# isabella232/kyverno

Hardware: AMD Instinct MI355X
Metric: resource×rule validate evals/sec (node) (higher is better)
Workload: dtype u8; 1 GPU; C2: synthetic Pods x 100 validate.pattern rules (image globs, ?*, quantities, |-lists); rules=100, pairs_per_gpu=100000000, output=full, parallelism=resource-shard x1, engine=specialized

## Files before the change

### kyverno_amd/csrc/kvdevfn.h

```cpp
#pragma once

#define KV_SENT 0xFFFFFFFFu


#ifdef KV_JIT_PRELUDE
#define KV_FN __device__ __forceinline__
#define KV_GLOB_FN __device__ __forceinline__
#else
#define KV_FN __device__
#define KV_GLOB_FN __device__ __noinline__
#endif

__device__ __forceinline__ uint32_t uni(uint32_t v) { return __builtin_amdgcn_readfirstlane(v); }

#ifndef KV_SCONST
#define KV_SCONST __attribute__((address_space(4)))
#endif
template <class T>
__device__ __forceinline__ T sld(const T* p) {
  static_assert(sizeof(T) % 4 == 0, "sld: whole words");
  const KV_SCONST uint32_t* q = (const KV_SCONST uint32_t*)p;
  uint32_t w[sizeof(T) / 4];
#pragma unroll
  for (uint32_t i = 0; i < sizeof(T) / 4; i++) w[i] = q[i];
// ... 576 lines not shown
  if (xm == 1) {
    for (uint32_t f = xf; f < xf + xc; f++)
      if (!(sld(P.fflags + f) & MF_EMPTY) && block_errs(P, B, R, rkind, rflags, f) == 0) return false;
    return true;
  }
  if (xm == 2) {
    for (uint32_t f = xf; f < xf + xc; f++)
      if ((sld(P.fflags + f) & MF_EMPTY) || block_errs(P, B, R, rkind, rflags, f) != 0) return true;
    return false;
  }
  if (!(sld(P.fflags + xf) & MF_EMPTY) && block_errs(P, B, R, rkind, rflags, xf) == 0) return false;
  return true;
}

__device__ __forceinline__ uint32_t wave_min(uint32_t v) {
#pragma unroll
  for (int o = 32; o >= 1; o >>= 1) {
    uint32_t x = __shfl_xor(v, o, 64);
    v = x < v ? x : v;
  }
  return v;
}


struct EState {
  uint32_t kind, flags, pn, key, res, i0, i1, i2, i3;
};

__device__ __forceinline__ uint2 err8_pack(uint32_t kind, uint32_t flags, uint32_t pn, uint32_t key, uint32_t i0,
                                           uint32_t i1, uint32_t i2, uint32_t i3, uint32_t r) {
  const uint32_t fits = (i0 < 1024u) & (i1 < 256u) & (i2 < 256u) & (i3 == 0u) & (key == ABSENT) & (pn < (1u << 25));
  uint2 w;
  w.x = kind | (flags << 4) | ((fits ^ 1u) << 6) | (pn << 7);
  w.y = (i0 & 1023u) | ((i1 & 255u) << 10) | ((i2 & 255u) << 18) | ((r & 63u) << 26);
  return w;
}

__device__ __forceinline__ void store_err(const DevOut& O, uint32_t ri, uint32_t n_res, uint32_t r, uint32_t kind,
                                          uint32_t flags, uint32_t pn, uint32_t key, uint32_t res, uint32_t i0,
                                          uint32_t i1, uint32_t i2, uint32_t i3) {
#if defined(KV_JIT_PRELUDE) && !defined(KVEMU)
  if (KV_OFULL(O) & 4) return;
#else
  if (KV_OFULL(O) & 4) {
    uint4* x = (uint4*)(O.err + (size_t)ri * n_res) + 2u * r;
    x[0] = make_uint4(kind | (flags << 16), pn, key, res);
    x[1] = make_uint4(i0, i1, i2, i3);
    return;
  }
#endif
  ((uint2*)(O.err8 + (size_t)ri * n_res))[r] = err8_pack(kind, flags, pn, key, i0, i1, i2, i3, r);
}

__device__ __forceinline__ uint32_t kv_count_bytes(uint32_t w, uint32_t b4) {
  const uint32_t t = w ^ b4;
  return (uint32_t)__popc(~(((t & 0x7F7F7F7Fu) + 0x7F7F7F7Fu) | t | 0x7F7F7F7Fu));
}

__device__ __forceinline__ uint32_t kv_ptab_col(uint32_t n_vals, uint32_t type, uint32_t a) {
  if (type - 1u < 4u) return a;
  return n_vals - KV_PTAB_PSEUDO + (type == NT_NULL ? 0u : type == NT_MAP ? 1u : 2u);
}
__device__ __forceinline__ uint32_t kv_ptab_col(const DevPS& P, uint32_t type, uint32_t a) {
  return kv_ptab_col(P.n_vals, type, a);
}

__device__ __forceinline__ uint32_t kv_arr_word(const uint32_t* __restrict__ ptab, uint32_t n_vals,
                                                const Node* __restrict__ N, uint32_t first, uint32_t count, uint32_t w) {
  uint32_t x = 0xFFFFFFFFu;
  for (uint32_t k = 0; k < count; k++) {
    const Node e = N[ni(first + k)];
    x &= kv_gld(ptab, (size_t)w * n_vals + kv_ptab_col(n_vals, node_type(e.kt), e.a));
  }
  return x;
}

__device__ __forceinline__ uint32_t kv_leaf_word(const DevPS& P, const Node* __restrict__ N, const Node& n, uint32_t w) {
  const uint32_t t = node_type(n.kt);
#ifdef KV_DIAG_XPTAB
  if (t != NT_ARR) return (n.a * 0x9E3779B9u) ^ (w * 0x85EBCA6Bu);
#endif
  if (t != NT_ARR) return kv_gld(P.ptab, (size_t)w * P.n_vals + kv_ptab_col(P, t, n.a));
  return kv_arr_word(P.ptab, P.n_vals, N, n.a, n.b, w);
}

__device__ __forceinline__ uint32_t kv_leaf_gather(const DevPS& P, const Node& n, uint32_t w) {
#ifdef KV_DIAG_XPTAB
  if (node_type(n.kt) != NT_ARR) return (n.a * 0x9E3779B9u) ^ (w * 0x85EBCA6Bu);
#endif
  return kv_gld(P.ptab, (size_t)w * P.n_vals + kv_ptab_col(P, node_type(n.kt), n.a));
}
__device__ __forceinline__ uint32_t kv_leaf_fix(const uint32_t* __restrict__ ptab, uint32_t n_vals, const Node* __restrict__ N,
                                             uint32_t a, uint32_t b, bool narrow, uint32_t w) {
  if (narrow) {
    const uint32_t ai = ni(a);
    a = kv_gld(&N[ai].a, 0);
    b = kv_gld(&N[ai].b, 0);
  }
  return kv_arr_word(ptab, n_vals, N, a, b, w);
}

__device__ __forceinline__ uint32_t kv_leaf_word_n(const DevPS& P, const Node* __restrict__ N, const Node& n, uint32_t w) {
  if (node_type(n.kt) != NT_ARR) return kv_leaf_word(P, N, n, w);
  return kv_leaf_fix(P.ptab, P.n_vals, N, n.a, 0u, true, w);
}

__device__ __forceinline__ void kv_rec_put(const DevOut& O, uint32_t ri, uint32_t n_res, uint32_t r, uint32_t slot,
                                           const EState& e, uint32_t z) {
#ifdef KV_DIAG_NORECST
  asm volatile("" ::"v"(slot));
  return;
// ... 92 lines not shown
    if (!((m >> j) & 1u)) continue;
    uint32_t ri = __builtin_amdgcn_readfirstlane(TB ? tab[j] : ri0 + j * sri);
    if (rec) {
      uint32_t z = 0u, rr = r;
      asm volatile("" : "+v"(rr), "+v"(z), "+s"(ri));
      const uint32_t ek = ekx ? ekx + ((TB ? tab[n + j] : j * spn) << 8) : 0u;
      const EState e{ek & 15u, (ek >> 4) & 15u, ek >> 8, ABSENT, ABSENT, i0, i1, i2, i3};
      if (slot) {
#if !defined(KV_DIAG_NORECST)
        ((uint2*)(O.err8 + (size_t)ri * n_res))[rr] = err8_pack(e.kind + z, e.flags, e.pn + z, e.key + z, e.i0, e.i1, e.i2, e.i3, rr);
#endif
      } else
        kv_rec_put(O, ri, n_res, rr, (uint32_t)(old[((row0 + j) >> 3) - w0] >> (8u * ((row0 + j) & 7u))) & 0xFFu, e, z);
    }
    s_row0[j * KV_RSTRIDE + threadIdx.x] = valid ? (uint8_t)st : (uint8_t)0xFFu;
  }
  }
#else
  for (uint32_t j = 0; j < n; j++) {
    if (!((m >> j) & 1u)) continue;
    const uint32_t ri = __builtin_amdgcn_readfirstlane(TB ? tab[j] : ri0 + j * sri);
    const uint32_t ek = ekx ? ekx + ((TB ? tab[n + j] : j * spn) << 8) : 0u;
    const EState e{ek & 15u, (ek >> 4) & 15u, ek >> 8, ABSENT, ABSENT, i0, i1, i2, i3};
    kv_final(O, ri, n_res, r, valid, st, e, s_row0 + j * KV_RSTRIDE, row0 + j);
  }
#endif
}

__device__ __forceinline__ void kv_wsync() {
#ifndef KVEMU
  __builtin_amdgcn_fence(__ATOMIC_RELEASE, "wavefront");
  __builtin_amdgcn_wave_barrier();
  __builtin_amdgcn_fence(__ATOMIC_ACQUIRE, "wavefront");
#endif
}

__device__ __forceinline__ void kv_prefill_rows(uint32_t* s_stw, uint32_t nr, uint32_t base, uint32_t n_res) {
  const uint32_t nv = n_res > base ? n_res - base : 0u;
#ifdef KVEMU
  for (uint32_t q = 0; q < nr; q++)
    ((uint8_t*)s_stw)[KV_ROW0 + q * KV_RSTRIDE + threadIdx.x] = threadIdx.x < nv ? (uint8_t)ST_NOMATCH : (uint8_t)0xFFu;
#else
  for (uint32_t t = threadIdx.x; t < KV_ROW0 / 4u; t += (uint32_t)KV_RWG) s_stw[t] = 0u;
  constexpr uint32_t WPR = KV_RSTRIDE / 4u;
  uint32_t* rows = s_stw + KV_ROW0 / 4u;
  const uint32_t k = threadIdx.x % WPR, l = k * 4u;
  uint32_t x = 0u;
  for (uint32_t j = 0u; j < 4u; j++) x |= (l + j < nv ? (uint32_t)ST_NOMATCH : 0xFFu) << (8u * j);
  for (uint32_t q = threadIdx.x / WPR; q < nr; q += (uint32_t)KV_RWG / WPR) rows[q * WPR + k] = x;
  __syncthreads();
#endif
}

__device__ __forceinline__ void kv_count_seg(const uint32_t* w, uint64_t m, uint32_t* c) {
  uint32_t c0 = 0u, c1 = 0u, c5 = 0u, cx = 0u, n = 0u;
#pragma unroll 4
  for (uint32_t i = 0; i < 16u; i++) {
    const uint32_t b = (uint32_t)(m >> (4u * i)) & 15u;
    const uint32_t keep = (((b * 0x00204081u) & 0x01010101u) * 0xFFu);
    const uint32_t x = (w[i] & keep) | (0xFEFEFEFEu & ~keep);
    c0 += kv_count_bytes(x, 0x00000000u);
    c1 += kv_count_bytes(x, 0x01010101u);
    c5 += kv_count_bytes(x, 0x05050505u);
    cx += kv_count_bytes(x, 0xFFFFFFFFu);
    n += (uint32_t)__popc(b);
  }
  for (uint32_t k = 0; k < (uint32_t)KV_HIST; k++) c[k] = 0u;
  c[ST_PASS] = c0;
  c[ST_FAIL] = c1;
  c[ST_NOMATCH] = c5;
  if (c0 + c1 + c5 + cx < n) {
    const uint32_t rest[4] = {ST_WARN, ST_ERROR, ST_SKIP, ST_CPU};
    for (uint32_t k = 0; k < 4u; k++) {
      uint32_t q = 0u;
      for (uint32_t i = 0; i < 16u; i++) {
        const uint32_t b = (uint32_t)(m >> (4u * i)) & 15u;
        const uint32_t keep = (((b * 0x00204081u) & 0x01010101u) * 0xFFu);
        q += kv_count_bytes((w[i] & keep) | (0xFEFEFEFEu & ~keep), rest[k] * 0x01010101u);
      }
      c[rest[k]] = q;
    }
  }
}

template <uint32_t NR>
__device__ __forceinline__ void kv_end_flush(const DevOut& O, uint32_t* s_stw, const uint32_t* rules,
                                             uint32_t n_res, uint32_t r, bool valid, uint32_t sc, uint32_t wsc,
                                             uint32_t n_rules) {
  constexpr uint32_t LPR = KV_RSTRIDE / 16u;
  constexpr uint32_t IPW = KV_KROWS / 4u;
  static_assert(NR >= 1u && NR <= KV_KROWS, "rows of one rule kernel");
  static_assert(KV_RSTRIDE % 16u == 0u && (uint32_t)KV_RWG % LPR == 0u && 64u % LPR == 0u, "a wave store writes whole rows");
  static_assert(LPR == 2u * (uint32_t)KV_HIST, "the copy loop and the sum loop walk the same rows");
  static_assert(KV_ROW0 == KV_RWAVES * KV_KROWS && KV_RWAVES * IPW >= KV_KROWS && IPW <= 64u,
                "the waves' counter bytes hold an id per row, each wave writing its own");
  const uint8_t* s_b = (const uint8_t*)s_stw + KV_ROW0;
#ifndef KVEMU
  const uint32_t* s_id = s_stw;
  {
    uint32_t t = (threadIdx.x >> 6) * IPW + (threadIdx.x & 63u);
    asm volatile("" : "+v"(t));
    uint32_t ri = kv_gld(rules, t < NR ? t : NR - 1u);
    asm volatile("" : "+v"(ri));
    if (KV_OFULL(O) & 8u) asm volatile("" : "+v"(sc));
    if ((threadIdx.x & 63u) < IPW && t < NR) s_stw[t] = ri;
  }
#endif
  __syncthreads();
#ifndef KVEMU
  const uint32_t wg0 = r - threadIdx.x;
#ifdef KV_DIAG_NOCOPY
  if (false) {
#else
  if ((KV_OFULL(O) & 1u) && wg0 + (uint32_t)KV_RWG <= n_res && (n_res & 15u) == 0u) {
#endif
    const uint32_t l = threadIdx.x & 63u, c16 = (threadIdx.x % LPR) * 16u;
    const size_t nwg = (n_res + (uint32_t)KV_RWG - 1u) / (uint32_t)KV_RWG;
    for (uint32_t q = threadIdx.x / LPR; q < NR; q += (uint32_t)KV_RWG / LPR) {
      const uint4 v = *(const uint4*)(s_b + q * KV_RSTRIDE + c16);
      const uint32_t ri = s_id[q];
      if (O.sflag) {
        constexpr uint32_t NM4 = 0x01010101u * (uint32_t)ST_NOMATCH;
        const bool nm = v.x == NM4 && v.y == NM4 && v.z == NM4 && v.w == NM4;
        const bool any = ((__ballot(!nm) >> (l & (64u - LPR))) & ((1ull << LPR) - 1ull)) != 0ull;
        if ((l % LPR) == 0u) O.sflag[(size_t)ri * nwg + wg0 / (uint32_t)KV_RWG] = any ? 1u : 0u;
        if (!any) continue;
      }
      *(uint4*)(O.status + (size_t)ri * n_res + wg0 + c16) = v;
    }
    __syncthreads();
  } else
#endif
  if ((KV_OFULL(O) & 1u) && valid) {
#pragma unroll 4
// ... 78 lines not shown
```

### kyverno_amd/csrc/kvjit.hpp

```cpp
#pragma once
#include <cstdint>
#include <map>
#include <string>
#include <vector>

#include "kvinternal.hpp"
#include "kvdevtypes.h"

namespace kvh {

struct JitChunk {
  std::vector<uint32_t> rules;
  std::string name;
};

struct JitKernelPlan {
  uint32_t first, count;
  int waves;
  std::vector<uint32_t> blocks;
  bool grouped = false;
  bool colloops = false;
};

struct JitImage {
  std::vector<JitKernelPlan> plan;
  std::string source;
  std::string common;
  std::vector<std::string> kernel_name, kernel_src;
  std::vector<std::vector<char>> codes;
  std::vector<JitChunk> chunks;
  std::vector<uint32_t> memo_preds;
  uint32_t memo_words = 0;
  uint32_t ptab_row = 1;
  uint32_t mtup_words = 0;
  std::vector<uint32_t> fac_word, fac_bit, fac_flist, fac_rule;
  uint32_t fac_slots = 0;
  std::vector<uint8_t> rec_compact;
  std::vector<uint32_t> gs_desc, gs_mem;
  uint32_t gs_members = 0;
  std::vector<kv::ColDesc> cols;
  std::vector<uint32_t> fam_arr, fam_parent, fam_ncols;
  std::vector<uint32_t> fam_nw, fam_nb, fam_nn;
  std::map<std::string, uint32_t> col_use;
  bool probe = false;
  double gen_ms = 0, compile_ms = 0;
  struct Variant {
    uint32_t full = 0;
    std::vector<std::vector<char>> codes;
  };
  std::vector<Variant> variants;
};

uint32_t jit_chunk_rules();
constexpr uint32_t kJitStamps = 16;
void jit_generate(const PolicySet& ps, uint32_t chunk_rules, JitImage* out);

void jit_build(const PolicySet& ps, JitImage* img);
uint64_t code_bytes(const JitImage& img);
struct RegVerdict {
  uint32_t priv, vgprs;
  bool calls;
  bool fits;
  bool scratch_ok;
  bool ships() const { return fits && scratch_ok; }
  bool probe_splits() const { return (priv != 0 && !calls) || !fits; }
};
RegVerdict reg_verdict_of(uint32_t priv, uint32_t vgprs, int waves, bool calls);
bool jit_plan_spills(JitImage* img, const std::vector<RegVerdict>& verdicts);
bool jit_load_plan(const std::string& key, JitImage* img);
void jit_save_plan(const std::string& key, const JitImage& img);

}
```

### kyverno_amd/csrc/kvjitbuild.cpp

```cpp
#include <hip/hiprtc.h>

#include <dlfcn.h>
#include <sched.h>
#include <spawn.h>
#include <sys/stat.h>
#include <sys/wait.h>

#include <cerrno>
#include <unistd.h>

#include <algorithm>
#include <atomic>
#include <chrono>
#include <cstdio>
#include <cstdlib>
#include <cstring>
#include <set>
#include <sstream>
#include <stdexcept>
#include <thread>

#include "kvjit.hpp"

extern char** environ;
// ... 216 lines not shown
  }
  unsigned T = std::min(16u, host_threads());
  if (const char* e = getenv("KVGPU_JIT_THREADS")) T = (unsigned)std::max(1, atoi(e));
  T = std::max(1u, std::min<unsigned>(T, (unsigned)todo.size()));
  const std::string jitc = jitc_path();
  const bool procs = !(getenv("KVGPU_JIT_PROCS") && getenv("KVGPU_JIT_PROCS")[0] == '0');
  if (!todo.empty() && procs && !jitc.empty() && todo.size() > 1) {
    compile_in_children(img, todo, jitc, T);
  } else {
    for (size_t i : todo) img->codes[i] = compile_one(img->common + img->kernel_src[i], img->kernel_name[i]);
  }
  if (!dir.empty())
    for (size_t i : todo) write_file_atomic(dir, paths[i], img->codes[i]);
  img->compile_ms += std::chrono::duration<double, std::milli>(std::chrono::steady_clock::now() - t0).count();
}

size_t program_of(const JitImage& img, const std::string& name) {
  return (size_t)(std::find(img.kernel_name.begin(), img.kernel_name.end(), name) - img.kernel_name.begin());
}

bool reg_verdict(const JitImage& img, size_t ci, int waves, RegVerdict* out) {
  uint32_t priv = 0, vgprs = 0;
  if (ci >= img.codes.size() || !co_kernel_info(img.codes[ci], img.kernel_name[ci], &priv, &vgprs)) return false;
  *out = reg_verdict_of(priv, vgprs, waves, img.kernel_src[ci].find("kv_dleaf_impl") != std::string::npos);
  return true;
}

std::string variant_common(const JitImage& img, uint32_t full) {
  return "#define KVJ_FULL " + std::to_string(full) + "u\n" + img.common;
}

}

RegVerdict reg_verdict_of(uint32_t priv, uint32_t vgprs, int waves, bool calls) {
  RegVerdict v{priv, vgprs, calls, false, false};
  v.fits = waves == 0 || vgprs <= 512u / (uint32_t)waves;
  v.scratch_ok = priv == 0 || (calls && waves == 0);
  return v;
}

bool jit_plan_spills(JitImage* img, const std::vector<RegVerdict>& verdicts) {
  std::vector<JitKernelPlan> next;
  bool changed = false;
  for (size_t k = 0; k < img->plan.size(); k++) {
    const JitKernelPlan& kp = img->plan[k];
    const RegVerdict& v = verdicts.at(k);
    if (v.ships()) {
      next.push_back(kp);
      continue;
    }
    changed = true;
    JitKernelPlan np = kp;
    const size_t big = (size_t)(std::max_element(np.blocks.begin(), np.blocks.end()) - np.blocks.begin());
    if (kp.colloops) {
      np.colloops = false;
    } else if (kp.grouped) {
      np.grouped = false;
    } else if (v.calls && v.fits) {
      np.waves = 0;
    } else if (kp.waves > 6 && np.blocks.size() > 1) {
      np.waves = kp.waves - 1;
    } else if (!np.blocks.empty() && np.blocks[big] > 1) {
      const uint32_t c = np.blocks[big], h = c / 2;
      np.blocks[big] = h;
      np.blocks.insert(np.blocks.begin() + big + 1, c - h);
    } else if (kp.waves > 1) {
      np.waves = kp.waves - 1;
    } else if (kp.waves == 1) {
      np.waves = 0;
    } else if (kp.count > 1) {
      const uint32_t h = kp.count / 2;
      next.push_back({kp.first, h, 0, std::vector<uint32_t>(h, 1u)});
      next.push_back({kp.first + h, kp.count - h, 0, std::vector<uint32_t>(kp.count - h, 1u)});
      continue;
    } else {
      throw std::runtime_error("kvjit: kernel " + img->chunks[k].name + " needs " + std::to_string(v.priv) +
                               " B of scratch per lane even without a launch bound");
    }
    next.push_back(np);
  }
  if (changed) img->plan = next;
  return changed;
}

namespace {

bool jit_plan_spills(JitImage* img) {
  std::vector<RegVerdict> verdicts(img->plan.size());
  for (size_t k = 0; k < img->plan.size(); k++)
    if (!reg_verdict(*img, program_of(*img, img->chunks[k].name), img->plan[k].waves, &verdicts[k]))
      throw std::runtime_error("kvjit: no kernel descriptor for " + img->chunks[k].name);
  return jit_plan_spills(img, verdicts);
}

void jit_compile_variants(JitImage* img) {
  img->variants.clear();
  for (uint32_t full : {3u, 8u}) {
    JitImage v;
    v.common = variant_common(*img, full);
    std::vector<size_t> at;
    for (size_t i = 0; i < img->kernel_name.size(); i++)
      if (img->kernel_name[i].rfind("kvj_r", 0) == 0) {
        v.kernel_name.push_back(img->kernel_name[i]);
        v.kernel_src.push_back(img->kernel_src[i]);
        at.push_back(i);
      }
    if (at.empty()) return;
// ... 30 lines not shown
      }
    }
    if (probe.plan.empty()) return;
    jit_generate(ps, chunk_rules, &probe);
    jit_compile(&probe);
    img->compile_ms += probe.compile_ms;
    std::set<std::pair<size_t, size_t>> split;
    for (size_t i = 0; i < probe.plan.size(); i++) {
      const std::string& name = probe.chunks[i].name;
      RegVerdict v;
      if (!reg_verdict(probe, program_of(probe, name), probe.plan[i].waves, &v))
        throw std::runtime_error("kvjit: no kernel descriptor for probe " + name);
      if (v.probe_splits()) split.insert(at[i]);
    }
    if (split.empty()) return;
    for (size_t k = 0; k < img->plan.size(); k++) {
      std::vector<uint32_t> nb;
      for (size_t b = 0; b < img->plan[k].blocks.size(); b++) {
        const uint32_t c = img->plan[k].blocks[b];
        if (split.count({k, b})) nb.insert(nb.end(), {c / 2, c - c / 2});
        else nb.push_back(c);
      }
      img->plan[k].blocks = nb;
    }
  }
}

std::string jit_plan_key(const JitImage& img) {
  uint64_t h = common_hash(img.common);
  for (size_t i = 0; i < img.kernel_src.size(); i++) h = fnv1a64(img.kernel_src[i], fnv1a64(img.kernel_name[i], h));
  char key[40];
  snprintf(key, sizeof key, "%016llx", (unsigned long long)h);
  return key;
}

}

uint64_t code_bytes(const JitImage& img) {
  uint64_t n = 0;
  for (auto& c : img.codes) n += c.size();
  return n;
}

bool jit_load_plan(const std::string& key, JitImage* img) {
  const std::string dir = cache_dir();
  std::vector<char> text;
  if (dir.empty() || !read_file(dir + "/plan-" + key + ".txt", &text)) return false;
  std::vector<JitKernelPlan> plan;
  std::istringstream in(std::string(text.begin(), text.end()));
  for (std::string line; std::getline(in, line);) {
    if (line.rfind("kernel ", 0) != 0) continue;
    std::istringstream ls(line.substr(7));
    JitKernelPlan kp{0, 0, 0, {}};
    ls >> kp.first >> kp.count >> kp.waves >> kp.grouped >> kp.colloops;
    uint32_t sum = 0;
    for (uint32_t b; ls >> b; sum += b) kp.blocks.push_back(b);
    if (sum != kp.count || kp.blocks.empty()) return false;
    plan.push_back(kp);
  }
  if (plan.empty()) return false;
  img->plan = plan;
  return true;
}

void jit_save_plan(const std::string& key, const JitImage& img) {
  const std::string dir = cache_dir();
  if (dir.empty()) return;
  std::string t;
  for (const JitKernelPlan& kp : img.plan) {
    t += "kernel " + std::to_string(kp.first) + " " + std::to_string(kp.count) + " " + std::to_string(kp.waves) + " " +
         (kp.grouped ? "1" : "0") + " " + (kp.colloops ? "1" : "0");
    for (uint32_t b : kp.blocks) t += " " + std::to_string(b);
    t += "\n";
  }
  const uint64_t hc = common_hash(img.common);
  for (size_t i = 0; i < img.kernel_src.size(); i++) t += "co " + cache_file(img, i, hc) + "\n";
  for (const JitImage::Variant& v : img.variants) {
    const uint64_t hv = common_hash(variant_common(img, v.full));
    for (size_t i = 0; i < img.kernel_src.size(); i++)
      if (i < v.codes.size() && !v.codes[i].empty()) t += "co " + cache_file(img, i, hv) + "\n";
  }
  write_file_atomic(dir, dir + "/plan-" + key + ".txt", t);
}

static void jit_group_regions(const PolicySet& ps, uint32_t chunk, JitImage* img) {
  static const bool kSteps[4][2] = {{true, true}, {true, false}, {false, true}, {false, false}};
  std::vector<int> step(img->plan.size(), 0);
  for (int round = 0; round < 4; round++) {
    for (size_t k = 0; k < img->plan.size(); k++) {
      img->plan[k].grouped = kSteps[step[k]][0];
      img->plan[k].colloops = kSteps[step[k]][1];
    }
    jit_generate(ps, chunk, img);
    jit_compile(img);
    bool back = false;
    for (size_t k = 0; k < img->plan.size(); k++) {
      RegVerdict v;
      if (!reg_verdict(*img, program_of(*img, img->chunks[k].name), img->plan[k].waves, &v))
        throw std::runtime_error("kvjit: no kernel descriptor for " + img->chunks[k].name);
      if (!v.ships() && step[k] < 3) {
        step[k]++;
        back = true;
      }
    }
    if (!back) return;
  }
}

void jit_build(const PolicySet& ps, JitImage* img) {
  const uint32_t chunk = jit_chunk_rules();
  const char* dump = getenv("KVGPU_JIT_DUMP");
  jit_generate(ps, chunk, img);
  if (dump) write_file(dump, img->source);
  if (!getenv("KVGPU_JIT_SKIP_COMPILE")) {
    const std::string pkey = jit_plan_key(*img);
    const bool stored = jit_load_plan(pkey, img);
    if (!stored) {
      for (JitKernelPlan& kp : img->plan) kp.grouped = kp.colloops = false;
      jit_refine_blocks(ps, chunk, img);
    }
    jit_generate(ps, chunk, img);
    bool settled = false;
    for (int round = 0; round < 64 && !settled; round++) {
      jit_compile(img);
      settled = !jit_plan_spills(img);
      if (!settled) jit_generate(ps, chunk, img);
    }
    if (!settled)
      throw std::runtime_error("kvjit: the register plan did not settle (kernels still spill after 64 re-plans)");
    if (!stored) jit_group_regions(ps, chunk, img);
    jit_compile_variants(img);
    jit_save_plan(pkey, *img);
    if (dump) write_file(dump, img->source);
  }
  if (const char* co = getenv("KVGPU_JIT_DUMP_CO")) {
    for (size_t i = 0; i < img->codes.size(); i++) write_file(std::string(co) + "." + img->kernel_name[i] + ".co", img->codes[i]);
    for (const JitImage::Variant& v : img->variants)
      for (size_t i = 0; i < v.codes.size(); i++)
        if (!v.codes[i].empty())
          write_file(std::string(co) + "." + img->kernel_name[i] + ".m" + std::to_string(v.full) + ".co", v.codes[i]);
  }
}

}
```

### kyverno_amd/csrc/kvjitgen.cpp

```cpp
#include <algorithm>
#include <chrono>
#include <cstdio>
#include <cstdlib>
#include <cstring>
#include <list>
#include <map>
#include <set>
#include <sstream>
#include <stdexcept>
#include <unordered_map>

#include "kvjit.hpp"
#include "kvdevtypes.h"

namespace kvh {

using namespace kv;

namespace {

const char* kPrelude =
#include "kvjit_prelude.inc"
    ;

std::string hex32(uint32_t v) {
  char b[16];
  snprintf(b, sizeof b, "0x%08xu", v);
  return b;
}
bool no_program(const RuleRec& rr) { return rr.route != 0 || rr.deny != 0; }
std::string u32(uint32_t v) { return std::to_string(v) + "u"; }
std::string u64(uint64_t v) { return std::to_string(v) + "ull"; }
std::string i64(int64_t v) {
  if (v == INT64_MIN) return "(-9223372036854775807ll - 1)";
  return std::to_string(v) + "ll";
}
std::string f64(double v) {
  uint64_t b;
  memcpy(&b, &v, 8);
  return "__longlong_as_double(" + i64((int64_t)b) + ")";
}

constexpr uint32_t kGslotMembers = 22u;

struct GenOpts {
  bool narrow, colloops, stamps, has_waves;
  int waves;
  uint32_t block_w;
  std::string diag;
  GenOpts() {
    const char* e = getenv("KVGPU_JIT_NARROW");
    narrow = !(e && e[0] == '0');
    e = getenv("KVGPU_JIT_COLLOOPS");
    colloops = !(e && e[0] == '0');
    stamps = getenv("KVGPU_JIT_STAMPS") != nullptr;
    e = getenv("KVGPU_JIT_WAVES");
    has_waves = e != nullptr;
    waves = e ? atoi(e) : 0;
    e = getenv("KVGPU_JIT_BLOCK_W");
    block_w = e && atoi(e) > 0 ? (uint32_t)atoi(e) : 0u;
    std::istringstream names((e = getenv("KVGPU_JIT_DIAG")) ? e : "");
    for (std::string t; std::getline(names, t, ',');)
      if (!t.empty()) diag += "#define KV_DIAG_" + t + " 1\n";
  }
};

struct Gen {
  struct Fam {
    std::string arr;
    uint32_t parent = 0, arr_j = 0;
    std::map<std::string, uint32_t> idx;
    std::vector<std::vector<uint32_t>> steps;
    std::vector<uint32_t> use;
  };
  struct Form {
    std::string text;
    std::vector<uint32_t> preds, pns;
    std::vector<uint32_t> leafpcs;
  };

  const PolicySet& ps;
  const GenOpts opt;

  std::vector<uint32_t> mpreds;
  std::map<uint32_t, uint32_t> pslot;
  std::map<uint32_t, uint32_t> pmask;
  std::vector<Fam> fams;
  std::map<std::string, uint32_t> fam_of;
  std::map<std::string, uint32_t> use_seed;
  std::vector<uint32_t> gs_desc, gs_mem;
  uint32_t gs_members = 0;
  std::vector<uint32_t> mt_bits;
  std::vector<uint8_t> rec_slot;
  uint32_t gtab_n = 0;
  std::map<uint32_t, Form> forms;
  std::map<uint32_t, uint32_t> bslot;
  std::map<uint32_t, std::set<uint32_t>> glob_bytes;
  std::vector<std::pair<std::string, std::string>> helpers;
  std::set<uint32_t> globs_done, atoms_done, preds_done, blks_done;
  std::set<std::pair<char, uint32_t>> qglobs_done, qatoms_done, qpreds_done;
  bool dleaf_done = false;
  std::vector<std::pair<std::string, std::string>> kernels;

  struct Kern {
    uint32_t mt_kbase = 0;
    uint32_t gs0 = 0, gsn = 0;
    std::string decls;
    bool grouped = false;
    bool colloops = false;
  };

  explicit Gen(const PolicySet& p) : ps(p), rec_slot(p.rules.size(), 0) {
    fams.emplace_back();
    col_of(0, "R");
  }

  struct Helper : std::ostringstream {
    Gen& g;
    const std::string name;
    Helper(Gen& gg, std::string n) : g(gg), name(std::move(n)) {}
    ~Helper() { g.helpers.push_back({name, str()}); }
  };
  static std::string num(const char* prefix, uint32_t i) { return prefix + std::to_string(i); }

  enum ColUse : uint32_t { CU_WIDE = 1u, CU_B = 2u, CU_LEAF = 4u };
  void col_mark(int fam, uint32_t j, uint32_t use) {
    if (fam >= 0 && j != kNoCol) fams.at((size_t)fam).use.at(j) |= use;
  }
  static std::string col_macro(const char* what, uint32_t f, uint32_t j) {
    return std::string("KVC_") + what + "_" + std::to_string(f) + "_" + std::to_string(j);
  }
  static constexpr uint32_t kNoCol = 0xFFFFFFFFu;
  static bool expr_steps(const std::string& ex, std::vector<uint32_t>* out) {
    out->clear();
    size_t at = ex.find('/');
    while (at != std::string::npos) {
      const size_t nx = ex.find('/', at + 1);
      const std::string tok = ex.substr(at + 1, nx == std::string::npos ? std::string::npos : nx - at - 1);
      if (tok.size() < 2 || (tok[0] != 's' && tok[0] != 'k')) return false;
      const unsigned long v = strtoul(tok.c_str() + 1, nullptr, 10);
      if (v >= KV_COL_SCAN) return false;
      out->push_back((uint32_t)v | (tok[0] == 'k' ? KV_COL_SCAN : 0u));
      at = nx;
    }
    return out->size() <= KV_COL_MAXD;
  }
  uint32_t col_of(uint32_t f, const std::string& rel) {
    Fam& F = fams.at(f);
    auto it = F.idx.find(rel);
    if (it != F.idx.end()) return it->second;
    std::vector<uint32_t> st;
    if (!expr_steps(rel, &st)) return kNoCol;
    const uint32_t j = (uint32_t)F.steps.size();
    F.idx.emplace(rel, j);
    F.steps.push_back(st);
    F.use.push_back(0u);
    return j;
  }
  uint32_t family(uint32_t parent, const std::string& rel) {
    if (parent && fams.at(parent).parent) return kNoCol;
    const std::string arr = parent ? fams[parent].arr + "[]" + rel : rel;
    auto it = fam_of.find(arr);
// ... 1454 lines not shown
    return "s_w + " + u32(KV_ROW0 + (B.hbase + q) * KV_RSTRIDE) + ", " + u32(B.hbase + q);
  }
  static std::string clear_err(const RGen& g) {
    std::string c = "ek" + g.s + " = 0u;";
    for (uint32_t lv = 0; lv <= g.max_level && lv < 4; lv++) c += " ei" + std::to_string(lv) + g.s + " = 0u;";
    if (g.uses_keyglob) c += " ekn" + g.s + " = ABSENT;";
    return c;
  }
  static std::string estate(const RGen* g, const std::string& ekx) {
    if (!g) return "EState e_{0u, 0u, 0u, ABSENT, ABSENT, 0u, 0u, 0u, 0u};";
    std::ostringstream k;
    k << "EState e_{" << ekx << " & 15u, (" << ekx << " >> 4) & 15u, " << ekx << " >> 8, "
      << (g->uses_keyglob ? "ekn" + g->s : std::string("ABSENT")) << ", ABSENT";
    for (uint32_t lv = 0; lv < 4; lv++) k << ", " << (lv <= g->max_level ? "ei" + std::to_string(lv) + g->s : "0u");
    k << "};";
    return k.str();
  }
  std::string store_st(const Block& B, uint32_t q, const RGen* g, const std::string& st, const std::string& ekx) const {
    std::ostringstream k;
    k << "  { " << estate(g, ekx) << "\n    kv_final(O, " << B.rules[q] << "u, n_res, r, valid, " << st << ", e_, "
      << row(B, q) << "); }\n";
    return k.str();
  }
  std::string store(const Block& B, uint32_t q) const {
    const RGen* g = B.at(q);
    const std::string s = g ? g->s : "_" + std::to_string(B.rules[q]);
    const std::string st = "rs" + s + " & 0xFFu";
    if (!g) return store_st(B, q, g, st, "0u");
    if (g->grp) return std::string();
    return "  if ((rs" + s + " & 0xFFu) != ST_STORED_ && (rs" + s + " & 0xFFu) != ST_NOMATCH) {\n" +
           store_st(B, q, g, st, "ek" + s) + "  }\n";
  }
  std::string match_code(const Block& B, uint32_t q) const {
    const RGen* g = B.at(q);
    return g && g->grp ? group_match_code(B, *g) : rule_match_code(B, q);
  }
  std::string group_match_code(const Block& B, const RGen& g) const {
    std::ostringstream k;
    const uint32_t p0 = B.kern.mt_kbase * 32u + g.grow, w0 = p0 / 32u, s0 = p0 % 32u;
    const uint32_t mask = g.gn >= 32 ? 0xFFFFFFFFu : (1u << g.gn) - 1u;
    k << "  { uint32_t mt_ = ((mw" << w0 << " >> " << s0 << "u)";
    if (s0 + g.gn > 32u) k << " | (mw" << (w0 + 1) << " << " << (32u - s0) << "u)";
    k << ") & " << hex32(mask) << ";\n";
    for (uint32_t j = 0; j < g.gn; j++)
      if (name_dependent(g.gri[j]))
        k << "    if (((mt_ >> " << j << "u) & 1u) && !g_match_" << g.gri[j] << "(P, B, R, rkind, rflags)) mt_ &= "
          << hex32(~(1u << j)) << ";\n";
    k << "    uint32_t cpu_ = (rflags & RF_MAGIC) ? mt_ : 0u;\n";
    for (uint32_t j = 0; j < g.gn; j++) {
      const RuleRec& rr = ps.rules[g.gri[j]];
      if (rr.flags & RR_META_EXPAND)
        k << "    cpu_ |= (rflags & " << u32(meta_bad_flags(rr.flags)) << ") ? (mt_ & " << u32(1u << j) << ") : 0u;\n";
    }
    for (uint32_t j = 0; j < g.gn; j++)
      k << "    s_w[" << u32(KV_ROW0 + (g.grow + j) * KV_RSTRIDE) << " + threadIdx.x] = valid ? (uint8_t)(((mt_ >> " << j
        << "u) & 1u) ? (((cpu_ >> " << j << "u) & 1u) ? ST_CPU : ST_PASS) : ST_NOMATCH) : (uint8_t)0xFFu;\n";
    k << "    al" << g.s << " = mt_ & ~cpu_; }\n";
    k << "  rs" << g.s << " = al" << g.s << " ? " << u32(g.b) << " : FIN_ | ST_STORED_;\n";
    return k.str();
  }
  std::string rule_match_code(const Block& B, uint32_t q) const {
    const uint32_t ri = B.rules[q];
    const RuleRec& rr = ps.rules[ri];
    const std::string s = "_" + std::to_string(ri);
    std::ostringstream k;
    k << "  if (" << mt_cond(B.kern, ri, B.hbase + q) << ") {\n";
    switch (rr.route) {
      case 1: k << "    rs" << s << " = FIN_ | ST_CPU;\n"; break;
      case 2: k << "    rs" << s << " = FIN_ | ST_NOMATCH;\n"; break;
      case 3: k << "    rs" << s << " = FIN_ | " << u32(rr.const_status) << ";\n"; break;
      default:
        k << "    if (rflags & RF_MAGIC) rs" << s << " = FIN_ | ST_CPU;\n";
        if (rr.flags & RR_META_EXPAND)
          k << "    else if (rflags & " << u32(meta_bad_flags(rr.flags)) << ") rs" << s << " = FIN_ | ST_CPU;\n";
        if (rr.pre)
          k << "    else if (B.pre_st[(size_t)" << (rr.pre - 1) << "u * n_res + r]) rs" << s << " = FIN_ | B.pre_st[(size_t)"
            << (rr.pre - 1) << "u * n_res + r];\n";
        if (rr.dyn)
          k << "    else if (B.dyn_st[(size_t)" << (rr.dyn - 1) << "u * n_res + r]) rs" << s << " = FIN_ | B.dyn_st[(size_t)"
            << (rr.dyn - 1) << "u * n_res + r];\n";
        if (rr.deny)
          k << "    else rs" << s << " = FIN_ | B.deny_st[(size_t)" << (rr.deny - 1) << "u * n_res + r];\n";
        else
          k << "    else rs" << s << " = " << u32(rr.prog) << ";\n";
        break;
    }
    k << "  }\n";
    return k.str();
  }

  static std::pair<uint32_t, uint32_t> segment(const RGen& g, size_t k) {
    return {k == 0 ? g.b : g.loops[k - 1].second + 1, k < g.loops.size() ? g.loops[k].first + 1 : g.e + 1};
  }

  struct LeanDecision {
    bool lean = false;
    bool alt = false;
    PostChain post;
    std::set<uint32_t> okset;
    std::vector<std::pair<uint32_t, PostChain>> errc;
    std::set<uint32_t> carry_ok, carry_err;
  };
  LeanDecision lean_decision(const RGen& g, size_t k, const std::set<uint32_t>& jumps,
                             const std::set<uint32_t>& err_jumps) const {
    LeanDecision D;
    const uint32_t se = segment(g, k).second, le = g.loops[k].second;
    D.post = post_chain(g, ps.prog[le].c);
    D.okset = jumps;
    std::set<uint32_t> errset = err_jumps;
// ... 203 lines not shown
      for (uint32_t d = 1; d < g.maxd; d++) k << ", c" << d << s << " = ABSENT";
      k << ";\n";
      k << "  uint32_t";
      for (uint32_t l = 0; l <= g.max_level && l < 4; l++)
        k << (l ? "," : "") << " li" << l << s << " = 0u, lf" << l << s << " = 0u, ll" << l << s << " = 0u";
      k << ";\n";
    }
  }

  static void check_resumes(const Block& B) {
    for (const RGen& g : B.gs)
      for (uint32_t t : g.resume) {
        bool ok = false;
        for (size_t k = 0; k <= g.loops.size() && !ok; k++) ok = t >= segment(g, k).first && t < segment(g, k).second;
        if (!ok) throw std::runtime_error("kvjit: resume target " + std::to_string(t) + " of rule " +
                                         std::to_string(g.ri) + " is not in a segment");
      }
  }

  std::string fused_block(Kern& kern, const std::vector<uint32_t>& rules_in, uint32_t hbase, std::vector<uint32_t>* order) {
    Block B(kern, hbase);
    form_groups(rules_in, &B);
    *order = B.rules;
    prepare_rules(&B);
    std::ostringstream body;
    for (size_t k = 0; k <= B.K; k++) {
      std::ostringstream seg;
      for (RGen& g : B.gs)
        if (k <= g.loops.size()) emit_segment(B, g, k, seg);
      if (k < B.K) {
        body << "  uint32_t";
        for (uint32_t w = 0; w < B.mask_words(); w++)
          body << (w ? "," : "") << " am" << k << "_" << w << " = 0u, sk" << k << "_" << w << " = 0u";
        body << ";\n";
      }
      body << B.global.flush(B.kern.grouped) << seg.str();
      if (k < B.K) emit_fused_loops(B, k, body);
    }
    check_resumes(B);
    std::ostringstream k;
    emit_rule_state(B, k);
    for (uint32_t q = 0; q < B.rules.size(); q++)
      if (no_program(ps.rules[B.rules[q]])) k << match_code(B, q) << store(B, q);
    k << body.str();
    return k.str();
  }

  static uint32_t kernel_lds(uint32_t nr) { return KV_ROW0 + nr * KV_RSTRIDE; }
  static int lds_waves(uint32_t nr) {
    const uint32_t g = 1280u, b = (kernel_lds(nr) + g - 1u) / g * g;
    return (int)std::max<uint32_t>(1u, (160u * 1024u) / std::max(b, g) * KV_RWAVES / 4u);
  }
  std::vector<uint32_t> group_kernel(const std::string& name, const std::vector<std::vector<uint32_t>>& chs, int waves,
                                     bool grouped, bool colloops) {
    std::vector<std::string> blocks;
    std::vector<std::pair<uint32_t, uint32_t>> rows;
    std::vector<uint32_t> rules;
    uint32_t nr_all = 0;
    for (const auto& c : chs) nr_all += (uint32_t)c.size();
    if (nr_all > KV_KROWS) throw std::runtime_error("kvjit: at most KV_KROWS rules per kernel (KVGPU_JIT_CHUNK)");
    Kern kern;
    kern.mt_kbase = (uint32_t)(mt_bits.size() / 32u);
    kern.gs0 = (uint32_t)(gs_desc.size() / 4u);
    kern.grouped = grouped;
    kern.colloops = colloops;
    for (const auto& c : chs) {
      std::vector<uint32_t> ord;
      rows.push_back({(uint32_t)rules.size(), (uint32_t)c.size()});
      blocks.push_back(fused_block(kern, c, (uint32_t)rules.size(), &ord));
      rules.insert(rules.end(), ord.begin(), ord.end());
    }
    mt_bits.insert(mt_bits.end(), rules.begin(), rules.end());
    while (mt_bits.size() % 32u) mt_bits.push_back(0xFFFFFFFFu);
    const uint32_t nr = (uint32_t)rules.size();
    if (kern.gsn > 64u) throw std::runtime_error("kvjit: more than 64 site-record groups in one kernel");
    std::ostringstream o;
    o << kern.decls;
    if (opt.stamps) o << "__device__ unsigned long long* kvj_stamps;\n";
    o << "__device__ const uint32_t " << name << "_rules[" << nr << "] = {";
    for (uint32_t q = 0; q < nr; q++) o << (q ? ", " : "") << u32(rules[q]);
    o << "};\n";
    const std::string lb = waves > 0 ? "KV_RWG, " + std::to_string(waves) : "KV_RWG";
    o << "extern \"C\" __global__ __launch_bounds__(" << lb << ") void " << name
      << "(const DevPS* __restrict__ Pp, const DevBatch* __restrict__ Bp, const Node* __restrict__ N, "
         "const Val* __restrict__ V, const uint8_t* __restrict__ S, DevOut O, uint32_t r0) {\n"
      << "  constexpr uint32_t FIN_ = " << u32(FIN) << ", ACT_ = " << u32(ACT) << ", ST_STORED_ = 0x7Eu;\n"
      << "  __shared__ unsigned long long s_stq[" << kernel_lds(nr) / 8 + (KV_RWAVES * kern.gsn + 1u) / 2u
      << "];\n  uint32_t* s_stw = (uint32_t*)s_stq;\n"
      << "  const DevPS& P = *Pp;\n  const DevBatch& B = *Bp;\n  const uint8_t* __restrict__ pstr = P.pstr;\n";
    o << "  const uint32_t nb_ = gridDim.x, x_ = blockIdx.x & 7u, per_ = nb_ >> 3, rem_ = nb_ & 7u;\n"
      << "  const uint32_t bx_ = x_ * per_ + (x_ < rem_ ? x_ : rem_) + (blockIdx.x >> 3);\n";
    o << "  const uint32_t r = r0 + bx_ * KV_RWG + threadIdx.x;\n"
      << "  const uint32_t n_res = B.n_res;\n"
      << "  const bool valid = r < n_res;\n"
      << "  const Res* __restrict__ R = B.res + (valid ? r : 0u);\n"
      << "  uint32_t root = ABSENT, rkind = KEY_NONE, rflags = 0u, rtup = 0u;\n"
      << "  if (valid) { root = ni(kv_gld(&R->root, 0)); rkind = kv_gld(&R->kind, 0); rflags = kv_gld(&R->flags, 0); rtup = kv_gld(&R->tup, 0); }\n"
      << "  Node rootn{0u, 0u, 0u, 0u};\n";
    o << "  const uint32_t* __restrict__ PC = B.pcol;\n"
        << "  const uint32_t ln_ = threadIdx.x & " << u32(KV_LANES - 1) << ", gw_ = (r >> 6) * KVC_W0;\n"
        << "  if (valid) rootn = " << col_macro("LD", 0, 0) << "(gw_);\n";
    o
      << "  const uint32_t* __restrict__ mtr_ = P.mtup + rtup;\n  const uint32_t ntup_ = B.n_tup;\n"
      << "  uint8_t* s_w = (uint8_t*)s_stw;\n"
      << "  uint32_t* const s_gc_ = s_stw + " << u32(kernel_lds(nr) / 4u) << ";\n"
      << (kern.gsn ? "  for (uint32_t t_ = threadIdx.x; t_ < " + u32(KV_RWAVES * kern.gsn) + "; t_ += KV_RWG) s_gc_[t_] = 0u;\n"
                : std::string())
      << "  kv_prefill_rows(s_stw, " << nr << "u, r - threadIdx.x, n_res);\n";
    auto stamp = [&](size_t k) {
      if (opt.stamps && k < kJitStamps)
        o << "  if (kvj_stamps && (threadIdx.x & 63u) == 0u) kvj_stamps[((size_t)blockIdx.x * KV_RWAVES + (threadIdx.x >> 6)) * "
          << kJitStamps << "u + " << k << "u] = __builtin_amdgcn_s_memtime();\n";
    };
    stamp(0);
    for (size_t bi = 0; bi < blocks.size(); bi++) {
      const uint32_t r0 = rows[bi].first, rn = rows[bi].second;
      const uint32_t p0 = kern.mt_kbase * 32u + r0, p1 = p0 + rn;
      o << "  {\n";
// ... 161 lines not shown
      case OP_INDEX:
        expr[d + 1].clear();
        break;
      default:
        break;
    }
  }
  std::sort(leaves.begin(), leaves.end());
  std::string sig = (arr.empty() ? "~" : arr) + "|";
  for (auto& l : leaves) sig += l + ",";
  return sig;
}

std::string rule_kind_key(const PolicySet& ps, uint32_t ri) {
  const RuleRec& rr = ps.rules[ri];
  std::vector<std::string> ks;
  for (uint32_t f = rr.m_first; f < rr.m_first + rr.m_count; f++) {
    const MFilter& F = ps.filters[f];
    if (!(F.flags & MF_KINDS)) return "*";
    for (uint32_t i = F.kinds_first; i < F.kinds_first + F.kinds_count; i++) {
      const KindSpec& k = ps.kinds[i];
      if (k.form == 3) return "*";
      ks.push_back(std::to_string(k.kind));
    }
  }
  std::sort(ks.begin(), ks.end());
  ks.erase(std::unique(ks.begin(), ks.end()), ks.end());
  std::string key;
  for (auto& k : ks) key += k + ",";
  return key;
}

std::vector<uint32_t> rule_order(const PolicySet& ps) {
  std::vector<std::pair<std::string, uint32_t>> order;
  for (uint32_t ri = 0; ri < ps.rules.size(); ri++)
    order.push_back({!no_program(ps.rules[ri]) ? "0" + rule_kind_key(ps, ri) + "#" + rule_signature(ps, ri) : "1", ri});
  std::stable_sort(order.begin(), order.end());
  std::vector<uint32_t> sorted;
  for (auto& o : order) sorted.push_back(o.second);
  return sorted;
}

std::vector<JitKernelPlan> first_plan(Gen& g, const std::vector<uint32_t>& sorted, uint32_t chunk_rules) {
  const uint32_t n = (uint32_t)sorted.size();
  if (chunk_rules == 0 || chunk_rules > KV_KROWS) chunk_rules = KV_KROWS;
  uint32_t parts = (n + chunk_rules - 1) / chunk_rules;
  while (parts < n && Gen::lds_waves((n + parts - 1) / parts) < Gen::lds_waves(n / parts)) parts++;
  std::vector<JitKernelPlan> plan;
  for (uint32_t k = 0; k < parts; k++) {
    const uint32_t a = (uint32_t)((uint64_t)n * k / parts), e = (uint32_t)((uint64_t)n * (k + 1) / parts);
    std::vector<uint32_t> bl = g.initial_blocks(sorted, a, e);
    const int lds_waves = Gen::lds_waves(e - a);
    const int rule_waves = (int)std::max<uint32_t>(1u, (160u * 1024u) / std::max<uint32_t>(1u, (e - a) * 256u));
    plan.push_back({a, e - a, g.opt.has_waves ? g.opt.waves : std::min({8, lds_waves, rule_waves}), bl, true, true});
  }
  return plan;
}

void assemble_programs(const Gen& g, const std::string& prelude, const std::string& cdefs, JitImage* out) {
  const std::vector<std::pair<std::string, std::string>>& defs = g.helpers;
  std::unordered_map<std::string, size_t> def_index;
  for (size_t i = 0; i < defs.size(); i++) def_index[defs[i].first] = i;
  auto refs = [&](const std::string& text, std::vector<size_t>* out_ids) {
    static const char* prefixes[] = {"g_glob_", "g_atom_", "g_pred_", "g_blk_", "g_match_",
                                     "g_dleaf_", "q_glob_", "q_atom_", "q_pred_", "r_glob_", "r_atom_", "r_pred_"};
    for (const char* pf : prefixes) {
      const size_t pl = strlen(pf);
      for (size_t q = text.find(pf); q != std::string::npos; q = text.find(pf, q + pl)) {
        size_t e = q + pl;
        while (e < text.size() && isdigit((unsigned char)text[e])) e++;
        auto it = def_index.find(text.substr(q, e - q));
        if (it != def_index.end()) out_ids->push_back(it->second);
      }
    }
  };
  out->common = prelude;
  out->kernel_name.clear();
  out->kernel_src.clear();
  out->source = prelude + cdefs;
  for (const auto& d : defs) out->source += d.second;
  for (auto& k : g.kernels) {
    std::vector<char> used(defs.size(), 0);
    std::vector<size_t> stack;
    refs(k.second, &stack);
    while (!stack.empty()) {
      const size_t d = stack.back();
      stack.pop_back();
      if (used[d]) continue;
      used[d] = 1;
      refs(defs[d].second, &stack);
    }
    std::string prog;
    for (size_t d = 0; d < defs.size(); d++)
      if (used[d]) prog += defs[d].second;
    out->kernel_name.push_back(k.first);
    out->kernel_src.push_back(cdefs + prog + k.second);
    out->source += k.second;
  }
}

}

uint32_t jit_chunk_rules() {
  const char* ch = getenv("KVGPU_JIT_CHUNK");
  return ch && atoi(ch) > 0 ? std::min<uint32_t>((uint32_t)atoi(ch), KV_KROWS) : KV_KROWS;
}

void jit_generate(const PolicySet& ps, uint32_t chunk_rules, JitImage* out) {
  auto t0 = std::chrono::steady_clock::now();
  Gen g(ps);
  g.use_seed = out->col_use;
  const std::string prelude =
      g.opt.diag + kPrelude + std::string("\nusing namespace kv;\n\n") +
      "__device__ __noinline__ bool kv_dleaf_impl(const DevBatch& B, const Node* __restrict__ N, uint32_t dp, Node vn);\n\n";
  for (uint32_t ri = 0; ri < ps.rules.size(); ri++)
    if (!no_program(ps.rules[ri])) g.leaf_classes(ri);
  for (uint32_t ri = 0; ri < ps.rules.size(); ri++) g.match_fn(ri);
  out->chunks.clear();
  const uint32_t n = (uint32_t)ps.rules.size();
  const std::vector<uint32_t> sorted = rule_order(ps);
  if (out->plan.empty() && n) out->plan = first_plan(g, sorted, chunk_rules);
  for (const JitKernelPlan& kp : out->plan) {
    JitChunk kc;
    kc.name = "kvj_r" + std::to_string(kp.first) + "_" + std::to_string(kp.count) +
              (kp.blocks.size() > 1 ? "_b" + std::to_string(kp.blocks.size()) : "") + (kp.waves ? "" : "u");
    for (uint32_t q = kp.first; q < kp.first + kp.count; q++) kc.rules.push_back(sorted.at(q));
    std::vector<std::vector<uint32_t>> bl;
    uint32_t at = 0;
    for (uint32_t c : kp.blocks) {
      if (at + c > kp.count) break;
      bl.emplace_back(kc.rules.begin() + at, kc.rules.begin() + at + c);
      at += c;
    }
    if (at != kp.count) throw std::runtime_error("kvjit: kernel plan blocks do not cover its rules");
    kc.rules = g.group_kernel(kc.name, bl, kp.waves, kp.grouped, kp.colloops);
    out->chunks.push_back(kc);
  }
  out->mtup_words = (uint32_t)(g.mt_bits.size() / 32u);
  if (out->mtup_words && !out->probe) g.build_fac(out);
  out->rec_compact.assign(n, 1);
  for (uint32_t ri = 0; ri < n; ri++) out->rec_compact[ri] = g.rec_slot[ri] ? 0 : 1;
  out->gs_desc = g.gs_desc;
  out->gs_mem = g.gs_mem;
  out->gs_members = g.gs_members;
  std::string cdefs;
  g.col_plan(out, &cdefs);

  out->memo_preds.clear();
  out->memo_words = 0;
  if (!g.mpreds.empty() && !out->probe) {
    g.ptab_kernel();
    out->memo_preds = g.mpreds;
    out->memo_words = (uint32_t)((g.mpreds.size() + 31) / 32);
    out->ptab_row = g.ptab_row_out();
  }
  assemble_programs(g, prelude, cdefs, out);
  out->gen_ms = std::chrono::duration<double, std::milli>(std::chrono::steady_clock::now() - t0).count();
}

}
```

Baseline: 365.3 billion evals/s.

## Add wave-uniform vectorized row staging and bit-sliced status histogram counting

Introduces kv_stage_rows, which writes whole 16-byte vectors of status bytes per row when every lane in a wave has identical match/cpu masks, falling back to per-lane byte stores otherwise. It also rewrites kv_count_seg to bit-slice the low three bits of each status byte into three planes and count all seven histogram bins with popcounts, replacing the per-status byte-compare passes. A new ustage plan flag, an environment toggle and extra register-fit fallback rounds in the JIT build select the uniform path per kernel, at the cost of more compile iterations. The new counter assumes status codes fit in three bits and that masked-out bytes read as 0xFF.

```diff
diff --git a/kyverno_amd/csrc/kvdevfn.h b/kyverno_amd/csrc/kvdevfn.h
--- a/kyverno_amd/csrc/kvdevfn.h
+++ b/kyverno_amd/csrc/kvdevfn.h
@@ -652,11 +652,6 @@
   ((uint2*)(O.err8 + (size_t)ri * n_res))[r] = err8_pack(kind, flags, pn, key, i0, i1, i2, i3, r);
 }
 
-__device__ __forceinline__ uint32_t kv_count_bytes(uint32_t w, uint32_t b4) {
-  const uint32_t t = w ^ b4;
-  return (uint32_t)__popc(~(((t & 0x7F7F7F7Fu) + 0x7F7F7F7Fu) | t | 0x7F7F7F7Fu));
-}
-
 __device__ __forceinline__ uint32_t kv_ptab_col(uint32_t n_vals, uint32_t type, uint32_t a) {
   if (type - 1u < 4u) return a;
   return n_vals - KV_PTAB_PSEUDO + (type == NT_NULL ? 0u : type == NT_MAP ? 1u : 2u);
@@ -855,34 +850,56 @@
 #endif
 }
 
+template <bool UNI>
+__device__ __forceinline__ void kv_stage_rows(uint8_t* s_w, uint32_t row0, uint32_t gn, bool valid, uint32_t mt,
+                                              uint32_t cpu) {
+#ifndef KVEMU
+  if constexpr (UNI) {
+    const uint32_t mt0 = __builtin_amdgcn_readfirstlane(mt), cpu0 = __builtin_amdgcn_readfirstlane(cpu);
+    if (__ballot(valid && ((mt ^ mt0) | (cpu ^ cpu0)) == 0u) == ~0ull) {
+      const uint32_t l = threadIdx.x & 63u;
+      uint8_t* seg = s_w + KV_ROW0 + row0 * KV_RSTRIDE + (threadIdx.x & ~63u) + (l & 3u) * 16u;
+      for (uint32_t j0 = 0; j0 < gn; j0 += 16u) {
+        const uint32_t j = j0 + (l >> 2);
+        const uint32_t st = ((mt0 >> j) & 1u) ? (((cpu0 >> j) & 1u) ? ST_CPU : ST_PASS) : ST_NOMATCH;
+        const uint32_t x = st * 0x01010101u;
+        if (j < gn) *(uint4*)(seg + j * KV_RSTRIDE) = make_uint4(x, x, x, x);
+      }
+      kv_wsync();
+      return;
+    }
+  }
+#endif
+  for (uint32_t j = 0; j < gn; j++)
+    s_w[KV_ROW0 + (row0 + j) * KV_RSTRIDE + threadIdx.x] =
+        valid ? (uint8_t)(((mt >> j) & 1u) ? (((cpu >> j) & 1u) ? ST_CPU : ST_PASS) : ST_NOMATCH) : (uint8_t)0xFFu;
+}
+
 __device__ __forceinline__ void kv_count_seg(const uint32_t* w, uint64_t m, uint32_t* c) {
-  uint32_t c0 = 0u, c1 = 0u, c5 = 0u, cx = 0u, n = 0u;
-#pragma unroll 4
-  for (uint32_t i = 0; i < 16u; i++) {
-    const uint32_t b = (uint32_t)(m >> (4u * i)) & 15u;
-    const uint32_t keep = (((b * 0x00204081u) & 0x01010101u) * 0xFFu);
-    const uint32_t x = (w[i] & keep) | (0xFEFEFEFEu & ~keep);
-    c0 += kv_count_bytes(x, 0x00000000u);
-    c1 += kv_count_bytes(x, 0x01010101u);
-    c5 += kv_count_bytes(x, 0x05050505u);
-    cx += kv_count_bytes(x, 0xFFFFFFFFu);
-    n += (uint32_t)__popc(b);
-  }
   for (uint32_t k = 0; k < (uint32_t)KV_HIST; k++) c[k] = 0u;
-  c[ST_PASS] = c0;
-  c[ST_FAIL] = c1;
-  c[ST_NOMATCH] = c5;
-  if (c0 + c1 + c5 + cx < n) {
-    const uint32_t rest[4] = {ST_WARN, ST_ERROR, ST_SKIP, ST_CPU};
-    for (uint32_t k = 0; k < 4u; k++) {
-      uint32_t q = 0u;
-      for (uint32_t i = 0; i < 16u; i++) {
-        const uint32_t b = (uint32_t)(m >> (4u * i)) & 15u;
-        const uint32_t keep = (((b * 0x00204081u) & 0x01010101u) * 0xFFu);
-        q += kv_count_bytes((w[i] & keep) | (0xFEFEFEFEu & ~keep), rest[k] * 0x01010101u);
+#pragma unroll
+  for (uint32_t g = 0; g < 2u; g++) {
+    uint32_t p0 = 0u, p1 = 0u, p2 = 0u;
+#pragma unroll
+    for (uint32_t p = 0; p < 4u; p++) {
+      uint32_t x[2];
+#pragma unroll
+      for (uint32_t h = 0; h < 2u; h++) {
+        const uint32_t i = 8u * g + 2u * p + h;
+        x[h] = w[i];
+        if (m != ~0ull) {
+          const uint32_t b = (uint32_t)(m >> (4u * i)) & 15u;
+          x[h] |= ~(((b * 0x00204081u) & 0x01010101u) * 0xFFu);
+        }
       }
-      c[rest[k]] = q;
-    }
+      const uint32_t z = (x[0] & 0x07070707u) | ((x[1] & 0x07070707u) << 4);
+      p0 |= (z & 0x11111111u) << p;
+      p1 |= ((z >> 1) & 0x11111111u) << p;
+      p2 |= ((z >> 2) & 0x11111111u) << p;
+    }
+#pragma unroll
+    for (uint32_t s = 0; s < 7u; s++)
+      c[s] += (uint32_t)__popc(((s & 1u) ? p0 : ~p0) & ((s & 2u) ? p1 : ~p1) & ((s & 4u) ? p2 : ~p2));
   }
 }
 
diff --git a/kyverno_amd/csrc/kvjit.hpp b/kyverno_amd/csrc/kvjit.hpp
--- a/kyverno_amd/csrc/kvjit.hpp
+++ b/kyverno_amd/csrc/kvjit.hpp
@@ -20,6 +20,7 @@
   std::vector<uint32_t> blocks;
   bool grouped = false;
   bool colloops = false;
+  bool ustage = false;
 };
 
 struct JitImage {
diff --git a/kyverno_amd/csrc/kvjitbuild.cpp b/kyverno_amd/csrc/kvjitbuild.cpp
--- a/kyverno_amd/csrc/kvjitbuild.cpp
+++ b/kyverno_amd/csrc/kvjitbuild.cpp
@@ -292,7 +292,9 @@
     changed = true;
     JitKernelPlan np = kp;
     const size_t big = (size_t)(std::max_element(np.blocks.begin(), np.blocks.end()) - np.blocks.begin());
-    if (kp.colloops) {
+    if (kp.ustage) {
+      np.ustage = false;
+    } else if (kp.colloops) {
       np.colloops = false;
     } else if (kp.grouped) {
       np.grouped = false;
@@ -429,7 +431,7 @@
     if (line.rfind("kernel ", 0) != 0) continue;
     std::istringstream ls(line.substr(7));
     JitKernelPlan kp{0, 0, 0, {}};
-    ls >> kp.first >> kp.count >> kp.waves >> kp.grouped >> kp.colloops;
+    ls >> kp.first >> kp.count >> kp.waves >> kp.grouped >> kp.colloops >> kp.ustage;
     uint32_t sum = 0;
     for (uint32_t b; ls >> b; sum += b) kp.blocks.push_back(b);
     if (sum != kp.count || kp.blocks.empty()) return false;
@@ -446,7 +448,7 @@
   std::string t;
   for (const JitKernelPlan& kp : img.plan) {
     t += "kernel " + std::to_string(kp.first) + " " + std::to_string(kp.count) + " " + std::to_string(kp.waves) + " " +
-         (kp.grouped ? "1" : "0") + " " + (kp.colloops ? "1" : "0");
+         (kp.grouped ? "1" : "0") + " " + (kp.colloops ? "1" : "0") + " " + (kp.ustage ? "1" : "0");
     for (uint32_t b : kp.blocks) t += " " + std::to_string(b);
     t += "\n";
   }
@@ -461,27 +463,50 @@
 }
 
 static void jit_group_regions(const PolicySet& ps, uint32_t chunk, JitImage* img) {
-  static const bool kSteps[4][2] = {{true, true}, {true, false}, {false, true}, {false, false}};
+  constexpr int kLast = 4;
+  static const bool kSteps[kLast + 1][3] = {{true, true, true}, {true, true, false}, {true, false, false},
+                                            {false, true, false}, {false, false, false}};
+  auto ships = [&](size_t k) {
+    RegVerdict v;
+    if (!reg_verdict(*img, program_of(*img, img->chunks[k].name), img->plan[k].waves, &v))
+      throw std::runtime_error("kvjit: no kernel descriptor for " + img->chunks[k].name);
+    return v.ships();
+  };
+  auto build = [&] {
+    jit_generate(ps, chunk, img);
+    jit_compile(img);
+  };
   std::vector<int> step(img->plan.size(), 0);
-  for (int round = 0; round < 4; round++) {
+  for (int round = 0; round <= kLast; round++) {
     for (size_t k = 0; k < img->plan.size(); k++) {
       img->plan[k].grouped = kSteps[step[k]][0];
       img->plan[k].colloops = kSteps[step[k]][1];
-    }
-    jit_generate(ps, chunk, img);
-    jit_compile(img);
+      img->plan[k].ustage = kSteps[step[k]][2];
+    }
+    build();
     bool back = false;
-    for (size_t k = 0; k < img->plan.size(); k++) {
-      RegVerdict v;
-      if (!reg_verdict(*img, program_of(*img, img->chunks[k].name), img->plan[k].waves, &v))
-        throw std::runtime_error("kvjit: no kernel descriptor for " + img->chunks[k].name);
-      if (!v.ships() && step[k] < 3) {
+    for (size_t k = 0; k < img->plan.size(); k++)
+      if (!ships(k) && step[k] < kLast) {
         step[k]++;
         back = true;
       }
-    }
-    if (!back) return;
-  }
+    if (!back) break;
+  }
+  std::vector<size_t> again;
+  for (size_t k = 0; k < img->plan.size(); k++)
+    if (step[k] >= 2) {
+      img->plan[k].ustage = true;
+      again.push_back(k);
+    }
+  if (again.empty()) return;
+  build();
+  bool back = false;
+  for (size_t k : again)
+    if (!ships(k)) {
+      img->plan[k].ustage = false;
+      back = true;
+    }
+  if (back) build();
 }
 
 void jit_build(const PolicySet& ps, JitImage* img) {
@@ -493,7 +518,7 @@
     const std::string pkey = jit_plan_key(*img);
     const bool stored = jit_load_plan(pkey, img);
     if (!stored) {
-      for (JitKernelPlan& kp : img->plan) kp.grouped = kp.colloops = false;
+      for (JitKernelPlan& kp : img->plan) kp.grouped = kp.colloops = kp.ustage = false;
       jit_refine_blocks(ps, chunk, img);
     }
     jit_generate(ps, chunk, img);
diff --git a/kyverno_amd/csrc/kvjitgen.cpp b/kyverno_amd/csrc/kvjitgen.cpp
--- a/kyverno_amd/csrc/kvjitgen.cpp
+++ b/kyverno_amd/csrc/kvjitgen.cpp
@@ -44,7 +44,7 @@
 constexpr uint32_t kGslotMembers = 22u;
 
 struct GenOpts {
-  bool narrow, colloops, stamps, has_waves;
+  bool narrow, colloops, ustage, stamps, has_waves;
   int waves;
   uint32_t block_w;
   std::string diag;
@@ -53,6 +53,8 @@
     narrow = !(e && e[0] == '0');
     e = getenv("KVGPU_JIT_COLLOOPS");
     colloops = !(e && e[0] == '0');
+    e = getenv("KVGPU_JIT_USTAGE");
+    ustage = !(e && e[0] == '0');
     stamps = getenv("KVGPU_JIT_STAMPS") != nullptr;
     e = getenv("KVGPU_JIT_WAVES");
     has_waves = e != nullptr;
@@ -108,6 +110,7 @@
     std::string decls;
     bool grouped = false;
     bool colloops = false;
+    bool ustage = false;
   };
 
   explicit Gen(const PolicySet& p) : ps(p), rec_slot(p.rules.size(), 0) {
@@ -1668,9 +1671,8 @@
       if (rr.flags & RR_META_EXPAND)
         k << "    cpu_ |= (rflags & " << u32(meta_bad_flags(rr.flags)) << ") ? (mt_ & " << u32(1u << j) << ") : 0u;\n";
     }
-    for (uint32_t j = 0; j < g.gn; j++)
-      k << "    s_w[" << u32(KV_ROW0 + (g.grow + j) * KV_RSTRIDE) << " + threadIdx.x] = valid ? (uint8_t)(((mt_ >> " << j
-        << "u) & 1u) ? (((cpu_ >> " << j << "u) & 1u) ? ST_CPU : ST_PASS) : ST_NOMATCH) : (uint8_t)0xFFu;\n";
+    k << "    kv_stage_rows<" << (opt.ustage && B.kern.ustage ? "true" : "false") << ">(s_w, " << u32(g.grow) << ", " << u32(g.gn)
+      << ", valid, mt_, cpu_);\n";
     k << "    al" << g.s << " = mt_ & ~cpu_; }\n";
     k << "  rs" << g.s << " = al" << g.s << " ? " << u32(g.b) << " : FIN_ | ST_STORED_;\n";
     return k.str();
@@ -1980,7 +1982,7 @@
     return (int)std::max<uint32_t>(1u, (160u * 1024u) / std::max(b, g) * KV_RWAVES / 4u);
   }
   std::vector<uint32_t> group_kernel(const std::string& name, const std::vector<std::vector<uint32_t>>& chs, int waves,
-                                     bool grouped, bool colloops) {
+                                     bool grouped, bool colloops, bool ustage) {
     std::vector<std::string> blocks;
     std::vector<std::pair<uint32_t, uint32_t>> rows;
     std::vector<uint32_t> rules;
@@ -1992,6 +1994,7 @@
     kern.gs0 = (uint32_t)(gs_desc.size() / 4u);
     kern.grouped = grouped;
     kern.colloops = colloops;
+    kern.ustage = ustage;
     for (const auto& c : chs) {
       std::vector<uint32_t> ord;
       rows.push_back({(uint32_t)rules.size(), (uint32_t)c.size()});
@@ -2259,7 +2262,7 @@
     std::vector<uint32_t> bl = g.initial_blocks(sorted, a, e);
     const int lds_waves = Gen::lds_waves(e - a);
     const int rule_waves = (int)std::max<uint32_t>(1u, (160u * 1024u) / std::max<uint32_t>(1u, (e - a) * 256u));
-    plan.push_back({a, e - a, g.opt.has_waves ? g.opt.waves : std::min({8, lds_waves, rule_waves}), bl, true, true});
+    plan.push_back({a, e - a, g.opt.has_waves ? g.opt.waves : std::min({8, lds_waves, rule_waves}), bl, true, true, true});
   }
   return plan;
 }
@@ -2340,7 +2343,7 @@
       at += c;
     }
     if (at != kp.count) throw std::runtime_error("kvjit: kernel plan blocks do not cover its rules");
-    kc.rules = g.group_kernel(kc.name, bl, kp.waves, kp.grouped, kp.colloops);
+    kc.rules = g.group_kernel(kc.name, bl, kp.waves, kp.grouped, kp.colloops, kp.ustage);
     out->chunks.push_back(kc);
   }
   out->mtup_words = (uint32_t)(g.mt_bits.size() / 32u);
```

After: 357.8 billion evals/s. 2.0% lower.
